# mrinmoy-iitg/SM_HPSS_MTL

Measured on AMD Instinct MI355X. Metric: clips/sec HPSS+MTL-CNN fwd (1s@16kHz), higher is better.
Workload: dtype f32

## Files before the change

### sm_hpss_mtl_amd/csrc/smh_fusion.hip

```cpp
#include "smh_model.h"
#include "smh_tcn_heads.h"

using namespace smh_tcn;

namespace {

constexpr int kFWaves = 16;
constexpr int kMaxMt = kPS / 16;

__device__ __forceinline__ f32x4 mfma4(float a, float b, f32x4 c) { return __builtin_amdgcn_mfma_f32_16x16x4f32(a, b, c, 0, 0, 0); }

template <bool TRAIN>
__global__ void __launch_bounds__(64 * kFWaves) fusion_dense_kernel(TcnArgs ta, int N, int D, const float *__restrict__ xh,
                                                                 const float *__restrict__ xp, const float *__restrict__ bn,
                                                                 const float *__restrict__ WhA, const float *__restrict__ hp,
                                                                 float *__restrict__ out) {
    extern __shared__ float part[];
    float *pre = part + (size_t)kFWaves * 16 * kPS;
    const int wave = __builtin_amdgcn_readfirstlane(threadIdx.x >> 6), lane = threadIdx.x & 63;
    const int i = lane & 15, q = lane >> 4;
    const int n0 = blockIdx.x * 16, g_here = min(16, N - n0);
    const int half = D / 2, ld = 64 * ((ta.NH + 63) / 64), n_mt = (ta.NH + 15) / 16;
    const int nr = min(n0 + i, N - 1);
    const float *gam = bn, *bet = bn + D, *mmean = bn + 2 * D, *mvar = bn + 3 * D;
    f32x4 acc[kMaxMt];
#pragma unroll
    for (int mt = 0; mt < kMaxMt; ++mt) acc[mt] = f32x4{0.f, 0.f, 0.f, 0.f};
    for (int c = wave; c < D / 16; c += kFWaves) {
        const int k = c * 16 + 4 * q;
        f32x4 av;
        const f32x4 g = *reinterpret_cast<const f32x4 *>(gam + k), b = *reinterpret_cast<const f32x4 *>(bet + k);
        if constexpr (TRAIN) {
            const f32x4 xv = *reinterpret_cast<const f32x4 *>(xh + (size_t)nr * D + k);
#pragma unroll
            for (int u = 0; u < 4; ++u) av[u] = xv[u] * g[u] + b[u];
        } else {
            const float *src = k < half ? xh + (size_t)nr * half + k : xp + (size_t)nr * half + (k - half);
            const f32x4 xv = *reinterpret_cast<const f32x4 *>(src);
            const f32x4 mm = *reinterpret_cast<const f32x4 *>(mmean + k), mv = *reinterpret_cast<const f32x4 *>(mvar + k);
#pragma unroll
            for (int u = 0; u < 4; ++u) av[u] = (xv[u] - mm[u]) / sqrtf(mv[u] + kBnEps) * g[u] + b[u];
        }
        const f32x4 *wrow = reinterpret_cast<const f32x4 *>(WhA) + (size_t)(c * 4 + q) * ld + i;
#pragma unroll
        for (int mt = 0; mt < kMaxMt; ++mt) {
            if (mt < n_mt) {
                const f32x4 bv = wrow[16 * mt];
#pragma unroll
                for (int u = 0; u < 4; ++u) acc[mt] = mfma4(av[u], bv[u], acc[mt]);
            }
        }
    }
#pragma unroll
    for (int mt = 0; mt < kMaxMt; ++mt)
        if (mt < n_mt)
#pragma unroll
            for (int r = 0; r < 4; ++r) part[((size_t)wave * 16 + 4 * q + r) * kPS + 16 * mt + i] = acc[mt][r];
    __syncthreads();
    for (int e = threadIdx.x; e < 16 * kPS; e += blockDim.x) {
        const int o = e % kPS;
        float v = 0.f;
        if (o < 16 * n_mt)
            for (int w = 0; w < kFWaves; ++w) v += part[(size_t)w * 16 * kPS + e];
        pre[e] = v;
    }
    __syncthreads();
    const float *bh = WhA + (size_t)D * ld;
    if constexpr (TRAIN) {
        for (int e = threadIdx.x; e < g_here * kPS; e += blockDim.x) {
            const int o = e % kPS;
            out[(size_t)n0 * kPS + e] = o < ta.NH ? pre[e] + bh[o] : 0.f;
        }
    } else {
        heads_tail(ta, pre, bh, hp, out, n0, g_here);
    }
}

constexpr int kFSlice = 32;
struct FusedAct {
    const float *acts[2];
    int nslot, half;
    __device__ __forceinline__ float pre_relu(int n, int k) const {
        const int b = k >= half, kk = k - b * half;
        return acts[b][((size_t)n * nslot + nslot - 1) * half + kk];
    }
};

__global__ void __launch_bounds__(256) fusion_bn_part_kernel(FusedAct fa, int N, int D, double *__restrict__ part) {
    const int k = blockIdx.x * 256 + threadIdx.x, s = blockIdx.y;
    if (k >= D) return;
    double s1 = 0.0, s2 = 0.0;
    for (int n = s * kFSlice; n < min(N, (s + 1) * kFSlice); ++n) {
        const double x = fmaxf(fa.pre_relu(n, k), 0.f);
        s1 += x, s2 += x * x;
    }
    part[((size_t)s * D + k) * 2] = s1;
    part[((size_t)s * D + k) * 2 + 1] = s2;
}

__global__ void __launch_bounds__(256) fusion_bn_final_kernel(int N, int D, int n_slices, const double *__restrict__ part,
// ... 11 lines not shown
__global__ void __launch_bounds__(256) fusion_bn_apply_kernel(FusedAct fa, int N, int D, const float *__restrict__ bnstat,
                                                              const float *__restrict__ vec, float *__restrict__ xhat) {
    const size_t e = (size_t)blockIdx.x * 256 + threadIdx.x;
    if (e >= (size_t)N * D) return;
    const int n = (int)(e / D), k = (int)(e - (size_t)n * D);
    xhat[e] = (fmaxf(fa.pre_relu(n, k), 0.f) - bnstat[k]) * vec[k];
}

struct FusionHeadOffs {
    size_t head[kMaxHeads];
};
__global__ void __launch_bounds__(256) fusion_dwh_kernel(int N, int D, int n_classes, const float *__restrict__ xhat,
                                                         const float *__restrict__ bn, const float *__restrict__ dpre,
                                                         float *__restrict__ grad, size_t off_c3, FusionHeadOffs offs) {
    const int wave = __builtin_amdgcn_readfirstlane(threadIdx.x >> 6), lane = threadIdx.x & 63;
    const int i = lane & 15, q = lane >> 4;
    const int k0 = (blockIdx.x * 4 + wave) * 16;
    if (k0 >= D) return;
    const int grp = blockIdx.y;
    const int ocount = grp == 0 ? n_classes : kHidden, col0 = grp == 0 ? 0 : n_classes + (grp - 1) * kHidden;
    const bool col_ok = i < ocount;
    const float g = bn[k0 + i], b = bn[D + k0 + i];
    f32x4 acc0 = {0.f, 0.f, 0.f, 0.f}, acc1 = acc0;
    for (int n = 0; n < N; n += 8) {
        float av[2], bv[2];
#pragma unroll
        for (int u = 0; u < 2; ++u) {
            const int nn = n + 4 * u + q;
            const bool ok = nn < N;
            const int nc = ok ? nn : 0;
            av[u] = ok ? xhat[(size_t)nc * D + k0 + i] * g + b : 0.f;
            bv[u] = (ok && col_ok) ? dpre[(size_t)nc * kPS + col0 + i] : 0.f;
        }
        acc0 = mfma4(av[0], bv[0], acc0);
        acc1 = mfma4(av[1], bv[1], acc1);
    }
    acc0 += acc1;
    if (col_ok) {
        const size_t base = (grp == 0 ? off_c3 : offs.head[grp - 1]) + (size_t)(k0 + 4 * q) * ocount + i;
#pragma unroll
        for (int r = 0; r < 4; ++r) grad[base + (size_t)r * ocount] = acc0[r];
    }
}

__global__ void __launch_bounds__(256) fusion_dx_kernel(int N, int D, int NH, const float *__restrict__ WhA,
                                                        const float *__restrict__ dpre, const float *__restrict__ xhat,
                                                        float *__restrict__ dy, double *__restrict__ part) {
    __shared__ float dp[kFSlice * kPS];
    const int k = blockIdx.x * 256 + threadIdx.x, s = blockIdx.y;
    const int nlo = s * kFSlice, nn = min(N, nlo + kFSlice) - nlo;
    for (int e = threadIdx.x; e < nn * kPS; e += 256) dp[e] = dpre[(size_t)nlo * kPS + e];
    __syncthreads();
    if (k >= D) return;
    const int ld = 64 * ((NH + 63) / 64);
    const float *w = WhA + (size_t)(k / 4) * ld * 4 + (k % 4);
    float acc[kFSlice];
#pragma unroll
    for (int r = 0; r < kFSlice; ++r) acc[r] = 0.f;
    for (int o = 0; o < NH; ++o) {
        const float wv = w[(size_t)o * 4];
#pragma unroll
        for (int r = 0; r < kFSlice; ++r) acc[r] = fmaf(dp[r * kPS + o], wv, acc[r]);
    }
    double s1 = 0.0, s2 = 0.0;
#pragma unroll
    for (int r = 0; r < kFSlice; ++r)
        if (r < nn) {
            const size_t e = (size_t)(nlo + r) * D + k;
            dy[e] = acc[r];
            s1 += acc[r];
            s2 += (double)acc[r] * xhat[e];
        }
    part[((size_t)s * D + k) * 2] = s1;
    part[((size_t)s * D + k) * 2 + 1] = s2;
}

__global__ void __launch_bounds__(256) fusion_bn_bwd_final_kernel(int N, int D, int n_slices, const double *__restrict__ part,
                                                                  float *__restrict__ grad, size_t off_bn, float *__restrict__ vec) {
    const int k = blockIdx.x * 256 + threadIdx.x;
    if (k >= D) return;
    double s1 = 0.0, s2 = 0.0;
    for (int s = 0; s < n_slices; ++s) s1 += part[((size_t)s * D + k) * 2], s2 += part[((size_t)s * D + k) * 2 + 1];
    grad[off_bn + k] = (float)s2;
    grad[off_bn + D + k] = (float)s1;
    vec[D + k] = (float)(s1 / N);
    vec[2 * D + k] = (float)(s2 / N);
}

__global__ void __launch_bounds__(256) fusion_bn_bwd_apply_kernel(FusedAct fa, int N, int D, const float *__restrict__ bn,
                                                                  const float *__restrict__ vec, const float *__restrict__ dy,
                                                                  const float *__restrict__ xhat, float *__restrict__ gt) {
    const size_t e = (size_t)blockIdx.x * 256 + threadIdx.x;
    if (e >= (size_t)N * D) return;
    const int n = (int)(e / D), k = (int)(e - (size_t)n * D);
    const int b = k >= fa.half, kk = k - b * fa.half;
    const float g = bn[k] * vec[k] * (dy[e] - vec[D + k] - xhat[e] * vec[2 * D + k]);
    gt[((size_t)b * N + n) * fa.half + kk] = fa.pre_relu(n, k) > 0.f ? g : 0.f;
}

}

namespace smh_tcn {

void fusion_tail_args(const smh_model *m, TcnArgs *a) {
    *a = TcnArgs{};
    a->D = m->D, a->NH = m->NH, a->n_mt = m->n_mt, a->n_classes = m->cfg.n_classes, a->n_heads = m->n_heads, a->out_dim = m->out_dim;
    for (int i = 0; i < kMaxHeads; ++i) a->head_odim[i] = m->head_odim[i], a->head_sigmoid[i] = m->head_sigmoid[i];
// ... 167 lines not shown
```

### sm_hpss_mtl_amd/csrc/smh_model.h

```cpp
#pragma once
#include "smh_common.h"

namespace smh_tcn {

using f32x4 = __attribute__((ext_vector_type(4))) float;

constexpr int C = 32;
constexpr int SX = 36;
constexpr int kMaxHeads = 4;
constexpr int kHidden = 16;
constexpr int kMaxG = 16;
constexpr int kPS = 80;
constexpr float kNormEps = 1e-5f;
constexpr float kBnEps = 1e-3f;
constexpr int kCat = kHidden + 2;
constexpr int kCatTail = 4 * kHidden + 4 * kCat + kCat + 1;
constexpr int kBlockFloats = 24 * 2 * 64 + 8 * 2 * 64 + 32 + 32;

struct TcnArgs {
    int N, T, F, FQ, G, GRP, n_blocks, n_dil, vec_ok;
    int D, NH, n_mt, n_classes, n_heads, out_dim, skip_heads;
    int wlds;
    unsigned long long *trace;
    int tune;
    int *status;
    int spin_limit;
    int split_last;
    int from_x0;
    int x0_shift, x0_T;
    int head_odim[kMaxHeads];
    int head_sigmoid[kMaxHeads];
    int cascade;
    int single;
    int trunk_only;
    int x0_one;
    const float *pair_X, *pair_W0, *pair_Wb;
    float *pair_trunk;
    const float *pair_WhA, *pair_hp;
    float *pair_out;
    int *pair_status;
};

struct TrainIO {
    float *acts;
    const float *drop_tcn;
    float *pre;
    float *upre;
    int acts_last_only;
};

struct HeadsArgs {
    int N, D, NH, n_classes, n_heads, out_dim;
    int head_odim[kMaxHeads], head_sigmoid[kMaxHeads];
    float lw[kMaxHeads + 1];
    size_t goff_head[kMaxHeads];
    size_t goff_c3b;
    size_t hp_off[kMaxHeads];
    int ext_losses;
    int stamps;
};
int launch_heads_train(const HeadsArgs &a, const float *pre, const float *y, const float *hp, const float *drop, float *dpre,
                       float *dxh, float *grad, float *bnstat, float *losses, unsigned *ticket, hipStream_t st);
int launch_cascade_heads_train(const HeadsArgs &a, const float *pre, const float *y, const float *hp, const float *drop,
                               float *dpre, float *dxh, float *dr, float *grad, float *bnstat, float *losses, hipStream_t st);
int launch_single_head_train(const HeadsArgs &a, const float *pre, const float *y, float *dpre, float *grad, float *losses,
// ... 78 lines not shown
```

### sm_hpss_mtl_amd/csrc/smh_tcn.hip

```cpp
#include <algorithm>
#include <cmath>
#include <cstdlib>
#include <cstring>
#include <type_traits>
#include <vector>

#include "smh_model.h"
#include "smh_tcn_heads.h"

using namespace smh_tcn;

namespace {

__device__ __forceinline__ f32x4 mfma4(float a, float b, f32x4 c) {
    return __builtin_amdgcn_mfma_f32_16x16x4f32(a, b, c, 0, 0, 0);
}

__device__ __forceinline__ float quad_max(float v) {
    const unsigned u = __float_as_uint(v);
    const auto r32 = __builtin_amdgcn_permlane32_swap(u, u, false, false);
    const float a = fmaxf(__uint_as_float(r32[0]), __uint_as_float(r32[1]));
    const unsigned ua = __float_as_uint(a);
    const auto r16 = __builtin_amdgcn_permlane16_swap(ua, ua, false, false);
    return fmaxf(__uint_as_float(r16[0]), __uint_as_float(r16[1]));
// ... 747 lines not shown
                    }
                    staged = blk + 2;
                    stage_ring(staged, 0, 1);
                }
                one_task(LdsWeights{ws + (size_t)(blk & (kWeightRing - 1)) * kBlockFloats, lane, q});
            }
        }
        publish();
        xin = (a.n_blocks & 1) ? xb : xa;
        xout = (a.n_blocks & 1) ? xa : xb;
        if (tracing && blockIdx.x < 1024 && threadIdx.x == 0) {
            a.trace[4 * (2000 + blockIdx.x) + 2] = __builtin_amdgcn_s_memtime();
            a.trace[4 * (2000 + blockIdx.x) + 3] = __builtin_amdgcn_s_memrealtime();
        }
    } else if (a.wlds && MODE == kPrefetch) {
        BlockW w0, w1;
        stage(0);
        if (a.n_blocks > 1) stage(1);
        asm volatile("s_waitcnt vmcnt(0)" ::: "memory");
        __syncthreads();
        load_block_lds(w0, ws, lane, q);
        for (int blk = 0; blk < a.n_blocks; blk += 2) {
            asm volatile("s_waitcnt vmcnt(0)" ::: "memory");
            __syncthreads();
            if (blk + 2 < a.n_blocks) stage(blk + 2);
            const bool more1 = blk + 1 < a.n_blocks;
            one_block(blk, w0, WeightPrefetch{w1, ws + kBlockFloats, lane, q});
            if (!more1) break;
            asm volatile("s_waitcnt vmcnt(0)" ::: "memory");
            __syncthreads();
            if (blk + 3 < a.n_blocks) stage(blk + 3);
            one_block(blk + 1, w1, WeightPrefetch{w0, ws, lane, q});
        }
    } else {
        if (a.wlds) stage(0);
        BlockW w;
        for (int blk = 0; blk < a.n_blocks; ++blk) {
            if (a.wlds) {
                asm volatile("s_waitcnt vmcnt(0)" ::: "memory");
                __syncthreads();
                if (blk + 1 < a.n_blocks) stage(blk + 1);
                one_block(blk, w, WeightLoad{w, ws + (size_t)(blk & 1) * kBlockFloats, lane, q});
            } else {
                __syncthreads();
                load_block_lds(w, Wb + (size_t)blk * kBlockFloats, lane, q);
                one_block(blk, w, NoPrefetch());
            }
        }
    }
    if (MODE != kSkew && MODE != kSkew16 && tracing && blockIdx.x < 1024 && threadIdx.x == 0) {
        a.trace[4 * (2000 + blockIdx.x) + 2] = __builtin_amdgcn_s_memtime();
        a.trace[4 * (2000 + blockIdx.x) + 3] = __builtin_amdgcn_s_memrealtime();
    }
    __syncthreads();
    if constexpr (MODE != kSkew && MODE != kSkew16) save_acts(xin, a.n_blocks);
    if constexpr (TRAIN) __syncthreads();
    for (int i = threadIdx.x; i < GR * (C / 4); i += blockDim.x) {
        const int R = i >> 3, c4 = (i & 7) * 4;
        f32x4 v = *reinterpret_cast<const f32x4 *>(xin + (size_t)R * SX + c4);
#pragma unroll
        for (int r = 0; r < 4; ++r) v[r] = fmaxf(v[r], 0.f);
        *reinterpret_cast<f32x4 *>(xin + (size_t)R * SX + c4) = v;
        if (trunk) *reinterpret_cast<f32x4 *>(trunk + ((size_t)n0 * T + R) * C + c4) = v;
    }
    __syncthreads();

    bool gave_up = false;
    if constexpr (MODE == kSkew || MODE == kSkew16) gave_up = ((__attribute__((address_space(3))) volatile int *)(flagbase))[63] != 0;
    dense_and_heads<TRAIN>(a, xin, xout, WhA, hp, out, tio, n0, g_here);
    if (tracing && blockIdx.x < 256 && threadIdx.x == 0) a.trace[4 * 3000 + 2 * blockIdx.x + 1] = __builtin_amdgcn_s_memrealtime();
    if (gave_up) {
        __syncthreads();
        for (int i = threadIdx.x; i < (a.trunk_only ? 0 : g_here * a.out_dim); i += blockDim.x) out[(size_t)n0 * a.out_dim + i] = 0.f;
        if (threadIdx.x == 0 && status) atomicOr(status, 1);
    }
}

__global__ void repack_kernel(const float *__restrict__ flat, const int *__restrict__ map, float *__restrict__ dst, size_t n) {
    const size_t i = (size_t)blockIdx.x * blockDim.x + threadIdx.x;
    if (i < n) {
        const int m = map[i];
        dst[i] = m ? flat[m - 1] : 0.f;
    }
}

static void pack_host(const smh_model *m, const float *h, std::vector<float> &W0, std::vector<float> &Wb,
                      std::vector<float> &WhA, std::vector<float> &hp) {
    const int F = m->cfg.n_feat, FQ = m->FQ, D = m->D, NH = m->NH, ncls = m->cfg.n_classes;
    W0.assign(m->nW0, 0.f), Wb.assign(m->nWb, 0.f), WhA.assign(m->nWhA, 0.f), hp.assign(m->nhp, 0.f);
    std::vector<float> Wh((size_t)D * NH, 0.f), bhv((size_t)m->n_mt * 16, 0.f);
    const float *p = h;
    if (m->heads == SMH_HEADS_FUSION) {
        p += 2 * trunk_floats(m->cfg) + (size_t)4 * D;
    } else if (m->cfg.block_variant == 1) {
        p += trunk_floats_v2(m->cfg);
    } else {
    for (int s = 0; s < FQ; ++s)
        for (int mt = 0; mt < 2; ++mt)
            for (int lane = 0; lane < 64; ++lane) {
                const int q = lane >> 4, i = lane & 15, f = q * FQ + s;
                W0[((size_t)s * 2 + mt) * 64 + lane] = f < F ? p[(size_t)f * C + 16 * mt + i] : 0.f;
            }
    p += (size_t)F * C;
    std::memcpy(&W0[(size_t)FQ * 2 * 64], p, C * sizeof(float));
    p += C;
    for (int b = 0; b < m->n_blocks; ++b) {
        float *wb = &Wb[(size_t)b * kBlockFloats];
        const float *k1 = p;
        p += 3 * C * C;
        const float *b1 = p;
        p += C;
        const float *k2 = p;
        p += C * C;
        const float *b2 = p;
        p += C;
        for (int s = 0; s < 24; ++s)
            for (int mt = 0; mt < 2; ++mt)
                for (int lane = 0; lane < 64; ++lane) {
                    const int q = lane >> 4, i = lane & 15;
                    const int tap = s / 8, c = 8 * q + s % 8;
                    const int n = s * 2 + mt;
                    wb[(n / 4) * 256 + 4 * lane + n % 4] = k1[((size_t)tap * C + c) * C + 16 * mt + i];
                }
        for (int e = 0; e < 8; ++e)
            for (int mt = 0; mt < 2; ++mt)
                for (int lane = 0; lane < 64; ++lane) {
                    const int q = lane >> 4, i = lane & 15;
                    const int cin = 16 * (e / 4) + 4 * q + (e % 4);
                    const int n = 48 + e * 2 + mt;
                    wb[(n / 4) * 256 + 4 * lane + n % 4] = k2[(size_t)cin * C + 16 * mt + i];
                }
        std::memcpy(wb + 24 * 2 * 64 + 8 * 2 * 64, b1, C * sizeof(float));
        std::memcpy(wb + 24 * 2 * 64 + 8 * 2 * 64 + 32, b2, C * sizeof(float));
    }
    }
    const float *k3c = p;
    p += (size_t)D * ncls;
    const float *b3c = p;
    p += ncls;
    for (int i = 0; i < D; ++i)
        for (int c = 0; c < ncls; ++c) Wh[(size_t)i * NH + c] = k3c[(size_t)i * ncls + c];
    for (int c = 0; c < ncls; ++c) bhv[c] = b3c[c];
    float *php = hp.data();
    for (int hd = 0; hd < m->n_heads; ++hd) {
        const float *kd = p;
        p += (size_t)D * kHidden;
        const float *bd = p;
        p += kHidden;
        for (int i = 0; i < D; ++i)
            for (int c = 0; c < kHidden; ++c) Wh[(size_t)i * NH + ncls + hd * kHidden + c] = kd[(size_t)i * kHidden + c];
        for (int c = 0; c < kHidden; ++c) bhv[ncls + hd * kHidden + c] = bd[c];
        const size_t cnt = head_tail_floats(m, hd);
        std::memcpy(php, p, cnt * sizeof(float));
        php += cnt;
        p += cnt;
    }
    const int ld = 64 * ((NH + 63) / 64);
    for (int k = 0; k < D; ++k)
        for (int o = 0; o < NH; ++o) WhA[(size_t)(k / 4) * ld * 4 + (size_t)o * 4 + (k % 4)] = Wh[(size_t)k * NH + o];
    std::memcpy(&WhA[(size_t)D * ld], bhv.data(), bhv.size() * sizeof(float));
}

}

static unsigned long long *g_trace = nullptr;
static unsigned g_trace_launches = 0;
constexpr size_t kTraceWords = 4 * 4096;
extern "C" int smh_internal_tcn_trace(int enable, unsigned long long *host, size_t words) {
    if (enable && !g_trace) {
        if (hipMalloc((void **)&g_trace, 2 * kTraceWords * sizeof(unsigned long long)) != hipSuccess) return -1;
        (void)hipMemset(g_trace, 0, 2 * kTraceWords * sizeof(unsigned long long));
    }
    if (host && g_trace) {
        (void)hipDeviceSynchronize();
        if (hipMemcpy(host, g_trace, std::min(words, 2 * kTraceWords) * sizeof(unsigned long long), hipMemcpyDeviceToHost) != hipSuccess) return -1;
    }
    if (!enable && g_trace) {
        (void)hipFree(g_trace);
        g_trace = nullptr;
    }
    return 0;
}

namespace smh_tcn {

Offsets offsets(const smh_model *m) {
    Offsets o;
    const size_t F = m->cfg.n_feat, D = m->D, ncls = m->cfg.n_classes;
    size_t p = 0;
    for (int h = 0; h < kMaxHeads; ++h) o.head[h] = 0;
    o.w0_k = p, p += F * C;
    o.w0_b = p, p += C;
    o.blk0 = p, o.blk_stride = 3 * C * C + C + C * C + C;
    p += (size_t)m->n_blocks * o.blk_stride;
    if (m->heads == SMH_HEADS_FUSION) {
        o.trunk_p = p, p += trunk_floats(m->cfg);
        o.fbn = p, p += 4 * D;
    }
    o.c3_k = p, p += D * ncls;
    o.c3_b = p, p += ncls;
    for (int h = 0; h < m->n_heads; ++h) {
        o.head[h] = p;
        p += D * kHidden + kHidden + head_tail_floats(m, h);
    }
    return o;
}

int repack(smh_model *m, hipStream_t st) {
    m->version++;
    if (m->heads == SMH_HEADS_FUSION) {
// ... 164 lines not shown
    SMH_REQUIRE(heads != SMH_HEADS_SINGLE || cfg->block_variant == 0,
                "smh_model_create_heads: the single-task model is built for block_variant 0 (keras-tcn 2.3.x) only");
    SMH_REQUIRE(heads != SMH_HEADS_FUSION || cfg->block_variant == 0,
                "smh_model_create_heads: the intermediate-fusion model is built for block_variant 0 (keras-tcn 2.3.x) only");
    SMH_REQUIRE(cfg->nb_filters == C, "B3_MTL kernel is tiled for nb_filters=32 (got %d)", cfg->nb_filters);
    SMH_REQUIRE(cfg->kernel_size == 3, "B3_MTL kernel supports kernel_size=3 (got %d)", cfg->kernel_size);
    if (heads == SMH_HEADS_SINGLE)
        SMH_REQUIRE(cfg->n_classes == 2 || cfg->n_classes == 3 || cfg->n_classes == 5,
                    "smh_model_create_heads: a single-task model has n_classes 2, 3 or 5 (got %d)", cfg->n_classes);
    else
        SMH_REQUIRE(cfg->n_classes == 3 || cfg->n_classes == 5, "n_classes must be 3 or 5 (got %d)", cfg->n_classes);
    SMH_REQUIRE(cfg->n_feat >= 1 && cfg->patch_size >= 1 && cfg->patch_size <= 512, "bad n_feat/patch_size");
    SMH_REQUIRE(cfg->nb_stacks >= 1 && cfg->n_dilations >= 1 && cfg->n_dilations <= 16, "bad stacks/dilations");
    SMH_REQUIRE(smh_device_count() > 0, "no HIP device visible: libsmh has no CPU path");
    smh_model *m = new smh_model();
    m->cfg = *cfg;
    m->n_blocks = cfg->nb_stacks * cfg->n_dilations;
    m->heads = heads;
    for (int i = 0; i < kMaxHeads; ++i) m->head_cat[i] = 0, m->head_odim[i] = 0, m->head_sigmoid[i] = 0;
    if (heads == SMH_HEADS_SINGLE) {
        m->n_heads = 0;
    } else if (heads == SMH_HEADS_CASCADED) {
        m->n_heads = 3;
        const int od[3] = {1, 1, 2}, sg[3] = {1, 1, 0};
        for (int i = 0; i < 3; ++i) m->head_odim[i] = od[i], m->head_sigmoid[i] = sg[i];
        m->head_cat[0] = m->head_cat[1] = kCat;
    } else if (cfg->n_classes == 5) {
        m->n_heads = 4;
        const int od[4] = {1, 1, 1, 3}, sg[4] = {1, 1, 1, 0};
        for (int i = 0; i < 4; ++i) m->head_odim[i] = od[i], m->head_sigmoid[i] = sg[i];
    } else {
        m->n_heads = 3;
        const int od[3] = {1, 1, 2}, sg[3] = {1, 1, 0};
        for (int i = 0; i < 3; ++i) m->head_odim[i] = od[i], m->head_sigmoid[i] = sg[i];
    }
    m->D = cfg->patch_size * C * (heads == SMH_HEADS_FUSION ? 2 : 1);
    m->NH = cfg->n_classes + kHidden * m->n_heads;
    m->n_mt = (m->NH + 15) / 16;
    m->out_dim = cfg->n_classes;
    for (int i = 0; i < m->n_heads; ++i) m->out_dim += m->head_odim[i];
    m->FQ = (cfg->n_feat + 3) / 4;
    SMH_REQUIRE(cfg->block_variant == 0 || cfg->block_variant == 1, "block_variant must be 0 (keras-tcn 2.3.x) or 1 (>= 2.8)");
    size_t n = (size_t)cfg->n_feat * C + C;
    n += (size_t)m->n_blocks * (3 * C * C + C + C * C + C);
    if (cfg->block_variant == 1) n = trunk_floats_v2(*cfg);
    if (heads == SMH_HEADS_FUSION) n = 2 * trunk_floats(*cfg) + (size_t)4 * m->D;
    n += (size_t)m->D * cfg->n_classes + cfg->n_classes;
    for (int i = 0; i < m->n_heads; ++i) n += (size_t)m->D * kHidden + kHidden + head_tail_floats(m, i);
    m->n_params = n;
    SMH_REQUIRE(n < (1u << 24), "model too large for the float-encoded gather map");
    m->nW0 = (size_t)m->FQ * 2 * 64 + 32;
    m->nWb = (size_t)m->n_blocks * kBlockFloats;
    if (cfg->block_variant == 1 || heads == SMH_HEADS_FUSION) m->nW0 = m->nWb = 0;
    m->nWhA = (size_t)m->D * 64 * ((m->NH + 63) / 64) + (size_t)m->n_mt * 16;
    m->nhp = 0;
    for (int i = 0; i < m->n_heads; ++i) m->nhp += head_tail_floats(m, i);
    std::vector<float> iota(n), W0, Wb, WhA, hp;
    for (size_t i = 0; i < n; ++i) iota[i] = (float)(i + 1);
    pack_host(m, iota.data(), W0, Wb, WhA, hp);
    std::vector<int> map;
    map.reserve(m->nW0 + m->nWb + m->nWhA + m->nhp);
    for (auto *v : {&W0, &Wb, &WhA, &hp})
        for (float f : *v) map.push_back((int)f);
    const size_t npk = map.size();
    hipError_t e = hipMalloc((void **)&m->d_flat, n * sizeof(float));
    if (e == hipSuccess) e = hipMalloc((void **)&m->d_W0, npk * sizeof(float));
    if (e == hipSuccess) e = hipMalloc((void **)&m->d_map, npk * sizeof(int));
    if (e == hipSuccess) e = hipMemcpy(m->d_map, map.data(), npk * sizeof(int), hipMemcpyHostToDevice);
    if (e == hipSuccess) e = hipMemset(m->d_flat, 0, n * sizeof(float));
    if (e == hipSuccess) e = hipMalloc((void **)&m->d_status, sizeof(int));
    if (e == hipSuccess) e = hipMemset(m->d_status, 0, sizeof(int));
    if (e == hipSuccess && heads == SMH_HEADS_FUSION) e = hipMalloc((void **)&m->d_w0cat, (size_t)2 * cfg->n_feat * C * sizeof(float));
    if (e == hipSuccess && heads == SMH_HEADS_FUSION) e = hipMemset(m->d_w0cat, 0, (size_t)2 * cfg->n_feat * C * sizeof(float));
    if (e != hipSuccess) {
        smh_model_destroy(m);
        return smh::set_error(SMH_E_HIP, "smh_model_create: device allocation failed: %s", hipGetErrorString(e));
    }
    m->d_Wb = m->d_W0 + m->nW0;
    m->d_WhA = m->d_Wb + m->nWb;
    m->d_hp = m->d_WhA + m->nWhA;
    if (heads == SMH_HEADS_FUSION) {
        for (int b = 0; b < 2; ++b) {
            const int rc = smh_model_create_heads(cfg, SMH_HEADS_MTL, &m->trunk[b]);
            if (rc) {
                smh_model_destroy(m);
                return rc;
            }
        }
    }
    *out = m;
    return SMH_OK;
}

extern "C" void smh_model_destroy(smh_model *m) {
    if (!m) return;
    (void)hipFree(m->d_flat);
    (void)hipFree(m->d_W0);
    (void)hipFree(m->d_map);
    (void)hipFree(m->d_bf16);
    (void)hipFree(m->d_status);
    (void)hipFree(m->d_w0cat);
    smh_model_destroy(m->trunk[0]);
    smh_model_destroy(m->trunk[1]);
    delete m;
}

extern "C" int smh_model_status(smh_model *m, void *stream) {
// ... 225 lines not shown
```

### sm_hpss_mtl_amd/csrc/smh_tcn_heads.h

```cpp
#pragma once
#include <type_traits>

#include "smh_model.h"

namespace smh_tcn {

__device__ __forceinline__ void cascaded_r(const TcnArgs &a, const float *pp, const float *bh, const float *hp, float r[2]) {
    const float *ph = hp + 2 * kCatTail;
    const float *gamma = ph, *beta = ph + 16, *mean = ph + 32, *var = ph + 48, *wo = ph + 64, *bo = wo + 2 * kHidden;
    r[0] = bo[0], r[1] = bo[1];
#pragma unroll
    for (int i = 0; i < kHidden; ++i) {
        const int o = a.n_classes + 2 * kHidden + i;
        float v = pp[o] + bh[o];
        v = (v - mean[i]) / sqrtf(var[i] + kBnEps);
        v = fmaxf(v * gamma[i] + beta[i], 0.f);
        r[0] = fmaf(v, wo[2 * i], r[0]);
        r[1] = fmaf(v, wo[2 * i + 1], r[1]);
    }
}

__device__ __forceinline__ void cascaded_head(const TcnArgs &a, const float *pp, const float *bh, const float *hp, float *orow, int h) {
    float r[2];
    cascaded_r(a, pp, bh, hp, r);
// ... 38 lines not shown
        }
        const float *gamma = ph, *beta = ph + 16, *mean = ph + 32, *var = ph + 48, *wo = ph + 64;
        const int od = a.head_odim[h];
        const float *bo = wo + kHidden * od;
        float hid[kHidden];
#pragma unroll
        for (int i = 0; i < kHidden; ++i) {
            const int o = a.n_classes + h * kHidden + i;
            float v = pre[p * kPS + o] + bh[o];
            v = (v - mean[i]) / sqrtf(var[i] + kBnEps);
            v = v * gamma[i] + beta[i];
            hid[i] = fmaxf(v, 0.f);
        }
        for (int c = 0; c < od; ++c) {
            float s = bo[c];
#pragma unroll
            for (int i = 0; i < kHidden; ++i) s = fmaf(hid[i], wo[i * od + c], s);
            if (a.head_sigmoid[h]) s = 1.0f / (1.0f + expf(-s));
            out[(size_t)(n0 + p) * a.out_dim + col + c] = s;
        }
    } else if (tid >= 128 && tid < 128 + g_here) {
        const int p = tid - 128;
        float mxl = -INFINITY;
        for (int c = 0; c < a.n_classes; ++c) mxl = fmaxf(mxl, pre[p * kPS + c] + bh[c]);
        float den = 0.f;
        for (int c = 0; c < a.n_classes; ++c) den += expf(pre[p * kPS + c] + bh[c] - mxl);
        const int col = a.out_dim - a.n_classes;
        for (int c = 0; c < a.n_classes; ++c)
            out[(size_t)(n0 + p) * a.out_dim + col + c] = expf(pre[p * kPS + c] + bh[c] - mxl) / den;
    }
}

__device__ __forceinline__ void single_tail(const TcnArgs &a, const float *pre, const float *bh, float *__restrict__ out, int n0,
                                            int g_here) {
    const int p = threadIdx.x;
    if (p >= g_here) return;
    constexpr int kMaxC = 5;
    float z[kMaxC], mx = -INFINITY, den = 0.f;
#pragma unroll
    for (int c = 0; c < kMaxC; ++c) {
        z[c] = c < a.n_classes ? pre[p * kPS + c] + bh[c] : -INFINITY;
        mx = fmaxf(mx, z[c]);
    }
#pragma unroll
    for (int c = 0; c < kMaxC; ++c) {
        z[c] = c < a.n_classes ? expf(z[c] - mx) : 0.f;
        den += z[c];
    }
#pragma unroll
    for (int c = 0; c < kMaxC; ++c)
        if (c < a.n_classes) out[(size_t)(n0 + p) * a.out_dim + c] = z[c] / den;
}

template <bool TRAIN>
__device__ __forceinline__ void dense_and_heads(const TcnArgs &a, const float *xin, float *xout, const float *__restrict__ WhA,
                                                const float *__restrict__ hp, float *__restrict__ out, const TrainIO &tio,
                                                int n0, int g_here) {
    if (a.trunk_only) return;
    const int wave = threadIdx.x >> 6, lane = threadIdx.x & 63, nw = blockDim.x >> 6;
    const int T = a.T;
    const int OPL = (a.NH + 63) >> 6;
    const int ld = OPL * 64;
    constexpr int kDenseParts = 8;
    float *part = xout;
    float *pre = xout + (size_t)kDenseParts * 4 * ld;
    const int rpp = (T + kDenseParts - 1) / kDenseParts;
    auto dense_on_trunk = [&](auto opl_c) {
        constexpr int kOPL = decltype(opl_c)::value;
        for (int g0 = 0; g0 < g_here; g0 += 4) {
            const float *xg[4];
#pragma unroll
            for (int g = 0; g < 4; ++g) xg[g] = xin + (size_t)min(g0 + g, g_here - 1) * T * SX;
            for (int pt = wave; pt < kDenseParts; pt += nw) {
                const int t_lo = min(T, pt * rpp), t_hi = min(T, t_lo + rpp);
                float acc[4][kOPL];
#pragma unroll
                for (int g = 0; g < 4; ++g)
#pragma unroll
                    for (int p = 0; p < kOPL; ++p) acc[g][p] = 0.f;
                for (int t = t_lo; t < t_hi; ++t) {
                    const f32x4 *wrow = reinterpret_cast<const f32x4 *>(WhA) + (size_t)t * (C / 4) * ld + lane;
#pragma unroll 2
                    for (int c8 = 0; c8 < 4; ++c8) {
                        f32x4 wa[kOPL], wb[kOPL];
#pragma unroll
                        for (int p = 0; p < kOPL; ++p) {
                            wa[p] = wrow[(size_t)(2 * c8) * ld + 64 * p];
                            wb[p] = wrow[(size_t)(2 * c8 + 1) * ld + 64 * p];
                        }
#pragma unroll
                        for (int g = 0; g < 4; ++g) {
                            const f32x4 xa = *reinterpret_cast<const f32x4 *>(xg[g] + (size_t)t * SX + 8 * c8);
                            const f32x4 xb = *reinterpret_cast<const f32x4 *>(xg[g] + (size_t)t * SX + 8 * c8 + 4);
#pragma unroll
                            for (int c = 0; c < 4; ++c)
#pragma unroll
                                for (int p = 0; p < kOPL; ++p) {
                                    acc[g][p] = fmaf(xa[c], wa[p][c], acc[g][p]);
                                    acc[g][p] = fmaf(xb[c], wb[p][c], acc[g][p]);
                                }
                        }
                    }
                }
#pragma unroll
                for (int g = 0; g < 4; ++g)
#pragma unroll
                    for (int p = 0; p < kOPL; ++p) part[((size_t)pt * 4 + g) * ld + 64 * p + lane] = acc[g][p];
            }
            __syncthreads();
            for (int i = threadIdx.x; i < 4 * ld; i += blockDim.x) {
                const int g = i / ld, o = i - g * ld;
                if (g0 + g < g_here && o < kPS) {
                    float v = 0.f;
#pragma unroll
                    for (int pt = 0; pt < kDenseParts; ++pt) v += part[((size_t)pt * 4 + g) * ld + o];
                    pre[(g0 + g) * kPS + o] = v;
                }
            }
            __syncthreads();
        }
    };
    if (!a.skip_heads) {
        if (OPL == 1) dense_on_trunk(std::integral_constant<int, 1>{});
        else dense_on_trunk(std::integral_constant<int, 2>{});
    }
    const float *bh = WhA + (size_t)a.D * ld;
    if constexpr (TRAIN) {
        for (int i = threadIdx.x; i < g_here * kPS; i += blockDim.x) {
            const int p = i / kPS, o = i - p * kPS;
            tio.pre[(size_t)(n0 + p) * kPS + o] = o < a.NH ? pre[p * kPS + o] + bh[o] : 0.f;
        }
        return;
    }
    if (a.single) single_tail(a, pre, bh, out, n0, g_here);
    else heads_tail(a, pre, bh, hp, out, n0, g_here);
}

}
```

### sm_hpss_mtl_amd/csrc/smh_tcn_v2.hip

```cpp
#include <algorithm>
#include <cstdlib>

#include "smh_model.h"
#include "smh_tcn_heads.h"

using namespace smh_tcn;

namespace {

__device__ __forceinline__ f32x4 mfma4(float a, float b, f32x4 c) { return __builtin_amdgcn_mfma_f32_16x16x4f32(a, b, c, 0, 0, 0); }

struct ConvW {
    float w[24][2];
    f32x4 blo, bhi;
};

__device__ __forceinline__ void load_conv(ConvW &cw, const float *__restrict__ k, const float *__restrict__ b, int q, int i) {
#pragma unroll
    for (int tap = 0; tap < 3; ++tap)
#pragma unroll
        for (int s8 = 0; s8 < 8; ++s8) {
            const float *p = k + ((size_t)tap * C + 8 * q + s8) * C + i;
            cw.w[tap * 8 + s8][0] = p[0];
            cw.w[tap * 8 + s8][1] = p[16];
// ... 93 lines not shown
                }
            } else {
                const float *xr = X + ((size_t)(n0 + g) * T + t) * C + 4 * q;
#pragma unroll
                for (int r = 0; r < 4; ++r) s0[r] = xr[r], s1[r] = xr[16 + r];
            }
#pragma unroll
            for (int r = 0; r < 4; ++r) {
                s0[r] = fmaxf(s0[r] + fmaxf(y0[r], 0.f), 0.f);
                s1[r] = fmaxf(s1[r] + fmaxf(y1[r], 0.f), 0.f);
            }
            float *dst = xa + (size_t)R * SX + 4 * q;
            *reinterpret_cast<f32x4 *>(dst) = s0;
            *reinterpret_cast<f32x4 *>(dst + 16) = s1;
        }
    }
    for (int blk = 1; blk < a.n_blocks; ++blk) {
        const int d = 1 << (blk % a.n_dil);
        const float *k0 = flat + blk0_floats + (size_t)(blk - 1) * blk_floats;
        const float *k1 = k0 + 3 * C * C + C;
        ConvW cw;
        load_conv(cw, k0, k0 + 3 * C * C, q, j);
        __syncthreads();
        for (int u = wave; u < units; u += nw) {
            const int R = 16 * u + j, Rc = min(R, GR - 1);
            const int t = Rc % T;
            f32x4 y0, y1;
            conv_tile(cw, xa, Rc, t, d, T, ZR, q, y0, y1);
#pragma unroll
            for (int r = 0; r < 4; ++r) y0[r] = fmaxf(y0[r], 0.f), y1[r] = fmaxf(y1[r], 0.f);
            float *dst = ya + (size_t)R * SX + 4 * q;
            *reinterpret_cast<f32x4 *>(dst) = y0;
            *reinterpret_cast<f32x4 *>(dst + 16) = y1;
        }
        load_conv(cw, k1, k1 + 3 * C * C, q, j);
        __syncthreads();
        for (int u = wave; u < units; u += nw) {
            const int R = 16 * u + j, Rc = min(R, GR - 1);
            const int t = Rc % T;
            f32x4 y0, y1;
            conv_tile(cw, ya, Rc, t, d, T, ZR, q, y0, y1);
            float *xr = xa + (size_t)Rc * SX + 4 * q;
            f32x4 s0 = *reinterpret_cast<const f32x4 *>(xr), s1 = *reinterpret_cast<const f32x4 *>(xr + 16);
#pragma unroll
            for (int r = 0; r < 4; ++r) {
                s0[r] = fmaxf(s0[r] + fmaxf(y0[r], 0.f), 0.f);
                s1[r] = fmaxf(s1[r] + fmaxf(y1[r], 0.f), 0.f);
            }
            float *dst = xa + (size_t)R * SX + 4 * q;
            *reinterpret_cast<f32x4 *>(dst) = s0;
            *reinterpret_cast<f32x4 *>(dst + 16) = s1;
        }
    }
    __syncthreads();
    if (trunk)
        for (int i = threadIdx.x; i < GR * (C / 4); i += blockDim.x) {
            const int R = i >> 3, c4 = (i & 7) * 4;
            *reinterpret_cast<f32x4 *>(trunk + ((size_t)n0 * T + R) * C + c4) = *reinterpret_cast<const f32x4 *>(xa + (size_t)R * SX + c4);
        }
    TrainIO none{nullptr, nullptr, nullptr, nullptr};
    dense_and_heads<false>(a, xa, ya, WhA, hp, out, none, n0, g_here);
}

}

namespace smh_tcn {

int launch_forward_v2(const smh_model *m, const float *d_x, int N, float *d_out, float *d_trunk, hipStream_t st) {
    TcnArgs a;
    size_t lds;
    fill_args(m, N, &a, &lds);
    lds = sizeof(float) * 2 * (size_t)(a.GRP + 1) * SX;
    SMH_REQUIRE(lds <= 156 * 1024, "patch_size %d too long for the LDS-resident TCN", a.T);
    const dim3 grid((N + a.G - 1) / a.G), block(512);
    SMH_CHECK_HIP(hipFuncSetAttribute((const void *)b3mtl_forward_v2_kernel, hipFuncAttributeMaxDynamicSharedMemorySize, (int)lds));
    hipLaunchKernelGGL(b3mtl_forward_v2_kernel, grid, block, lds, st, a, d_x, (const float *)m->d_flat, (const float *)m->d_WhA,
                       (const float *)m->d_hp, d_trunk, d_out);
    return smh::launch_status("b3mtl_forward_v2_kernel");
}

}
```

Before: 2.663 million.

## Software-pipeline dense-head weight loads with buffer loads, prefetch ring and packed layout

```diff
diff --git a/sm_hpss_mtl_amd/csrc/smh_fusion.hip b/sm_hpss_mtl_amd/csrc/smh_fusion.hip
--- a/sm_hpss_mtl_amd/csrc/smh_fusion.hip
+++ b/sm_hpss_mtl_amd/csrc/smh_fusion.hip
@@ -20,7 +20,7 @@
     const int wave = __builtin_amdgcn_readfirstlane(threadIdx.x >> 6), lane = threadIdx.x & 63;
     const int i = lane & 15, q = lane >> 4;
     const int n0 = blockIdx.x * 16, g_here = min(16, N - n0);
-    const int half = D / 2, ld = 64 * ((ta.NH + 63) / 64), n_mt = (ta.NH + 15) / 16;
+    const int half = D / 2, ld = dense_ld(ta.NH), n_mt = (ta.NH + 15) / 16;
     const int nr = min(n0 + i, N - 1);
     const float *gam = bn, *bet = bn + D, *mmean = bn + 2 * D, *mvar = bn + 3 * D;
     f32x4 acc[kMaxMt];
@@ -41,11 +41,11 @@
 #pragma unroll
             for (int u = 0; u < 4; ++u) av[u] = (xv[u] - mm[u]) / sqrtf(mv[u] + kBnEps) * g[u] + b[u];
         }
-        const f32x4 *wrow = reinterpret_cast<const f32x4 *>(WhA) + (size_t)(c * 4 + q) * ld + i;
+        const f32x4 *wrow = reinterpret_cast<const f32x4 *>(WhA) + (size_t)(c * 4 + q) * ld;
 #pragma unroll
         for (int mt = 0; mt < kMaxMt; ++mt) {
             if (mt < n_mt) {
-                const f32x4 bv = wrow[16 * mt];
+                const f32x4 bv = wrow[min(16 * mt + i, ta.NH - 1)];
 #pragma unroll
                 for (int u = 0; u < 4; ++u) acc[mt] = mfma4(av[u], bv[u], acc[mt]);
             }
@@ -163,7 +163,7 @@
     for (int e = threadIdx.x; e < nn * kPS; e += 256) dp[e] = dpre[(size_t)nlo * kPS + e];
     __syncthreads();
     if (k >= D) return;
-    const int ld = 64 * ((NH + 63) / 64);
+    const int ld = dense_ld(NH);
     const float *w = WhA + (size_t)(k / 4) * ld * 4 + (k % 4);
     float acc[kFSlice];
 #pragma unroll
diff --git a/sm_hpss_mtl_amd/csrc/smh_model.h b/sm_hpss_mtl_amd/csrc/smh_model.h
--- a/sm_hpss_mtl_amd/csrc/smh_model.h
+++ b/sm_hpss_mtl_amd/csrc/smh_model.h
@@ -11,6 +11,7 @@
 constexpr int kHidden = 16;
 constexpr int kMaxG = 16;
 constexpr int kPS = 80;
+__host__ __device__ constexpr int dense_ld(int NH) { return (NH + 3) & ~3; }
 constexpr float kNormEps = 1e-5f;
 constexpr float kBnEps = 1e-3f;
 constexpr int kCat = kHidden + 2;
diff --git a/sm_hpss_mtl_amd/csrc/smh_tcn.hip b/sm_hpss_mtl_amd/csrc/smh_tcn.hip
--- a/sm_hpss_mtl_amd/csrc/smh_tcn.hip
+++ b/sm_hpss_mtl_amd/csrc/smh_tcn.hip
@@ -823,6 +823,9 @@
         a.trace[4 * (2000 + blockIdx.x) + 2] = __builtin_amdgcn_s_memtime();
         a.trace[4 * (2000 + blockIdx.x) + 3] = __builtin_amdgcn_s_memrealtime();
     }
+    constexpr int kRows = MODE == kOneSet ? 2 : kDenseRows;
+    DenseFirst<kRows> dense_first;
+    dense_prefetch(a, WhA, dense_first);
     __syncthreads();
     if constexpr (MODE != kSkew && MODE != kSkew16) save_acts(xin, a.n_blocks);
     if constexpr (TRAIN) __syncthreads();
@@ -838,7 +841,7 @@
 
     bool gave_up = false;
     if constexpr (MODE == kSkew || MODE == kSkew16) gave_up = ((__attribute__((address_space(3))) volatile int *)(flagbase))[63] != 0;
-    dense_and_heads<TRAIN>(a, xin, xout, WhA, hp, out, tio, n0, g_here);
+    dense_and_heads<TRAIN, kRows>(a, xin, xout, WhA, hp, out, tio, n0, g_here, dense_first);
     if (tracing && blockIdx.x < 256 && threadIdx.x == 0) a.trace[4 * 3000 + 2 * blockIdx.x + 1] = __builtin_amdgcn_s_memrealtime();
     if (gave_up) {
         __syncthreads();
@@ -926,7 +929,7 @@
         php += cnt;
         p += cnt;
     }
-    const int ld = 64 * ((NH + 63) / 64);
+    const int ld = dense_ld(NH);
     for (int k = 0; k < D; ++k)
         for (int o = 0; o < NH; ++o) WhA[(size_t)(k / 4) * ld * 4 + (size_t)o * 4 + (k % 4)] = Wh[(size_t)k * NH + o];
     std::memcpy(&WhA[(size_t)D * ld], bhv.data(), bhv.size() * sizeof(float));
@@ -1197,7 +1200,7 @@
     m->nW0 = (size_t)m->FQ * 2 * 64 + 32;
     m->nWb = (size_t)m->n_blocks * kBlockFloats;
     if (cfg->block_variant == 1 || heads == SMH_HEADS_FUSION) m->nW0 = m->nWb = 0;
-    m->nWhA = (size_t)m->D * 64 * ((m->NH + 63) / 64) + (size_t)m->n_mt * 16;
+    m->nWhA = (size_t)m->D * dense_ld(m->NH) + (size_t)m->n_mt * 16;
     m->nhp = 0;
     for (int i = 0; i < m->n_heads; ++i) m->nhp += head_tail_floats(m, i);
     std::vector<float> iota(n), W0, Wb, WhA, hp;
diff --git a/sm_hpss_mtl_amd/csrc/smh_tcn_heads.h b/sm_hpss_mtl_amd/csrc/smh_tcn_heads.h
--- a/sm_hpss_mtl_amd/csrc/smh_tcn_heads.h
+++ b/sm_hpss_mtl_amd/csrc/smh_tcn_heads.h
@@ -114,42 +114,104 @@
         if (c < a.n_classes) out[(size_t)(n0 + p) * a.out_dim + c] = z[c] / den;
 }
 
-template <bool TRAIN>
+constexpr int kDenseParts = 8;
+constexpr int kDenseRows = 8;
+
+template <int OPL, int ROWS>
+struct DenseRing {
+    f32x4 w[OPL][ROWS];
+};
+template <int ROWS>
+using DenseFirst = DenseRing<2, ROWS>;
+
+typedef unsigned u32x4 __attribute__((ext_vector_type(4)));
+__device__ __forceinline__ unsigned dense_col(int NH, int lane, int p) { return 16u * (unsigned)min(64 * p + lane, NH - 1); }
+__device__ __forceinline__ __amdgpu_buffer_rsrc_t dense_rsrc(const float *WhA, int D, int ldc) {
+    return __builtin_amdgcn_make_buffer_rsrc(const_cast<float *>(WhA), 0, 4u * (unsigned)D * (unsigned)ldc, 0x00020000);
+}
+template <int OPL, int ROWS, int N>
+__device__ __forceinline__ void dense_load_pair(f32x4 (&w)[N][ROWS], __amdgpu_buffer_rsrc_t rw, int ldc, int t, int c8,
+                                                const unsigned *coff) {
+    static_assert(ROWS == 2 || ROWS == 4 || ROWS == 8, "ring slots: 2, 4 or 8 rows");
+    const unsigned rowb = 16u * (unsigned)ldc;
+#pragma unroll
+    for (int r = 0; r < 2; ++r)
+#pragma unroll
+        for (int p = 0; p < OPL; ++p) {
+            const u32x4 v = __builtin_amdgcn_raw_buffer_load_b128(rw, coff[p], ((unsigned)t * (C / 4) + 2 * c8 + r) * rowb, 0);
+            w[p][(2 * c8 + r) % ROWS] = f32x4{__uint_as_float(v.x), __uint_as_float(v.y), __uint_as_float(v.z), __uint_as_float(v.w)};
+        }
+}
+
+__device__ __forceinline__ void dense_range(int T, int pt, int &t_lo, int &t_hi) {
+    const int rpp = (T + kDenseParts - 1) / kDenseParts;
+    t_lo = min(T, pt * rpp), t_hi = min(T, t_lo + rpp);
+}
+
+template <int ROWS>
+__device__ __forceinline__ void dense_prefetch(const TcnArgs &a, const float *__restrict__ WhA, DenseFirst<ROWS> &first) {
+    const int wave = __builtin_amdgcn_readfirstlane(threadIdx.x >> 6), lane = threadIdx.x & 63;
+    int t_lo, t_hi;
+    dense_range(a.T, wave, t_lo, t_hi);
+    if (a.trunk_only || a.skip_heads || wave >= kDenseParts || t_lo >= t_hi) return;
+    const unsigned col[2] = {dense_col(a.NH, lane, 0), dense_col(a.NH, lane, 1)};
+    const int ldc = dense_ld(a.NH);
+    const __amdgpu_buffer_rsrc_t rw = dense_rsrc(WhA, a.D, ldc);
+    if (a.NH <= 64) {
+#pragma unroll
+        for (int c8 = 0; c8 < ROWS / 2; ++c8) dense_load_pair<1>(first.w, rw, ldc, t_lo, c8, col);
+    } else {
+#pragma unroll
+        for (int c8 = 0; c8 < ROWS / 2; ++c8) dense_load_pair<2>(first.w, rw, ldc, t_lo, c8, col);
+    }
+}
+
+template <bool TRAIN, int ROWS>
 __device__ __forceinline__ void dense_and_heads(const TcnArgs &a, const float *xin, float *xout, const float *__restrict__ WhA,
                                                 const float *__restrict__ hp, float *__restrict__ out, const TrainIO &tio,
-                                                int n0, int g_here) {
+                                                int n0, int g_here, const DenseFirst<ROWS> &first) {
     if (a.trunk_only) return;
-    const int wave = threadIdx.x >> 6, lane = threadIdx.x & 63, nw = blockDim.x >> 6;
+    const int wave = __builtin_amdgcn_readfirstlane(threadIdx.x >> 6), lane = threadIdx.x & 63, nw = blockDim.x >> 6;
     const int T = a.T;
     const int OPL = (a.NH + 63) >> 6;
-    const int ld = OPL * 64;
-    constexpr int kDenseParts = 8;
+    const int ldc = dense_ld(a.NH);
+    const int pl = OPL * 64;
     float *part = xout;
-    float *pre = xout + (size_t)kDenseParts * 4 * ld;
-    const int rpp = (T + kDenseParts - 1) / kDenseParts;
+    float *pre = xout + (size_t)kDenseParts * 4 * pl;
+    const __amdgpu_buffer_rsrc_t rw = dense_rsrc(WhA, a.D, ldc);
     auto dense_on_trunk = [&](auto opl_c) {
         constexpr int kOPL = decltype(opl_c)::value;
+        unsigned col[kOPL];
+#pragma unroll
+        for (int p = 0; p < kOPL; ++p) col[p] = dense_col(a.NH, lane, p);
+        DenseRing<kOPL, ROWS> f;
+#pragma unroll
+        for (int p = 0; p < kOPL; ++p)
+#pragma unroll
+            for (int h = 0; h < ROWS; ++h) f.w[p][h] = first.w[p][h];
         for (int g0 = 0; g0 < g_here; g0 += 4) {
             const float *xg[4];
 #pragma unroll
             for (int g = 0; g < 4; ++g) xg[g] = xin + (size_t)min(g0 + g, g_here - 1) * T * SX;
             for (int pt = wave; pt < kDenseParts; pt += nw) {
-                const int t_lo = min(T, pt * rpp), t_hi = min(T, t_lo + rpp);
+                int t_lo, t_hi;
+                dense_range(T, pt, t_lo, t_hi);
+                int t_next = -1;
+                {
+                    int npt = pt + nw, ng0 = g0, n_lo, n_hi;
+                    if (npt >= kDenseParts) npt = wave, ng0 = g0 + 4;
+                    dense_range(T, npt, n_lo, n_hi);
+                    if (ng0 < g_here && n_lo < n_hi) t_next = n_lo;
+                }
                 float acc[4][kOPL];
 #pragma unroll
                 for (int g = 0; g < 4; ++g)
 #pragma unroll
                     for (int p = 0; p < kOPL; ++p) acc[g][p] = 0.f;
-                for (int t = t_lo; t < t_hi; ++t) {
-                    const f32x4 *wrow = reinterpret_cast<const f32x4 *>(WhA) + (size_t)t * (C / 4) * ld + lane;
-#pragma unroll 2
+                auto frame = [&](int t, int nt, auto more_c) {
+                    constexpr bool MORE = decltype(more_c)::value;
+#pragma unroll
                     for (int c8 = 0; c8 < 4; ++c8) {
-                        f32x4 wa[kOPL], wb[kOPL];
-#pragma unroll
-                        for (int p = 0; p < kOPL; ++p) {
-                            wa[p] = wrow[(size_t)(2 * c8) * ld + 64 * p];
-                            wb[p] = wrow[(size_t)(2 * c8 + 1) * ld + 64 * p];
-                        }
 #pragma unroll
                         for (int g = 0; g < 4; ++g) {
                             const f32x4 xa = *reinterpret_cast<const f32x4 *>(xg[g] + (size_t)t * SX + 8 * c8);
@@ -158,24 +220,36 @@
                             for (int c = 0; c < 4; ++c)
 #pragma unroll
                                 for (int p = 0; p < kOPL; ++p) {
-                                    acc[g][p] = fmaf(xa[c], wa[p][c], acc[g][p]);
-                                    acc[g][p] = fmaf(xb[c], wb[p][c], acc[g][p]);
+                                    acc[g][p] = fmaf(xa[c], f.w[p][(2 * c8) % ROWS][c], acc[g][p]);
+                                    acc[g][p] = fmaf(xb[c], f.w[p][(2 * c8 + 1) % ROWS][c], acc[g][p]);
                                 }
                         }
+                        const int c8n = (c8 + ROWS / 2) & 3;
+                        const bool same = c8 + ROWS / 2 < 4;
+                        if (same || MORE) {
+                            __builtin_amdgcn_sched_barrier(0);
+                            dense_load_pair<kOPL>(f.w, rw, ldc, same ? t : nt, c8n, col);
+                            __builtin_amdgcn_sched_barrier(0);
+                        }
                     }
+                };
+                for (int t = t_lo; t + 1 < t_hi; ++t) frame(t, t + 1, std::true_type{});
+                if (t_lo < t_hi) {
+                    if (t_next >= 0) frame(t_hi - 1, t_next, std::true_type{});
+                    else frame(t_hi - 1, -1, std::false_type{});
                 }
 #pragma unroll
                 for (int g = 0; g < 4; ++g)
 #pragma unroll
-                    for (int p = 0; p < kOPL; ++p) part[((size_t)pt * 4 + g) * ld + 64 * p + lane] = acc[g][p];
+                    for (int p = 0; p < kOPL; ++p) part[((size_t)pt * 4 + g) * pl + 64 * p + lane] = acc[g][p];
             }
             __syncthreads();
-            for (int i = threadIdx.x; i < 4 * ld; i += blockDim.x) {
-                const int g = i / ld, o = i - g * ld;
+            for (int i = threadIdx.x; i < 4 * pl; i += blockDim.x) {
+                const int g = i / pl, o = i - g * pl;
                 if (g0 + g < g_here && o < kPS) {
                     float v = 0.f;
 #pragma unroll
-                    for (int pt = 0; pt < kDenseParts; ++pt) v += part[((size_t)pt * 4 + g) * ld + o];
+                    for (int pt = 0; pt < kDenseParts; ++pt) v += part[((size_t)pt * 4 + g) * pl + o];
                     pre[(g0 + g) * kPS + o] = v;
                 }
             }
@@ -186,7 +260,7 @@
         if (OPL == 1) dense_on_trunk(std::integral_constant<int, 1>{});
         else dense_on_trunk(std::integral_constant<int, 2>{});
     }
-    const float *bh = WhA + (size_t)a.D * ld;
+    const float *bh = WhA + (size_t)a.D * ldc;
     if constexpr (TRAIN) {
         for (int i = threadIdx.x; i < g_here * kPS; i += blockDim.x) {
             const int p = i / kPS, o = i - p * kPS;
diff --git a/sm_hpss_mtl_amd/csrc/smh_tcn_v2.hip b/sm_hpss_mtl_amd/csrc/smh_tcn_v2.hip
--- a/sm_hpss_mtl_amd/csrc/smh_tcn_v2.hip
+++ b/sm_hpss_mtl_amd/csrc/smh_tcn_v2.hip
@@ -169,6 +169,8 @@
             *reinterpret_cast<f32x4 *>(dst + 16) = s1;
         }
     }
+    DenseFirst<kDenseRows> dense_first;
+    dense_prefetch(a, WhA, dense_first);
     __syncthreads();
     if (trunk)
         for (int i = threadIdx.x; i < GR * (C / 4); i += blockDim.x) {
@@ -176,7 +178,7 @@
             *reinterpret_cast<f32x4 *>(trunk + ((size_t)n0 * T + R) * C + c4) = *reinterpret_cast<const f32x4 *>(xa + (size_t)R * SX + c4);
         }
     TrainIO none{nullptr, nullptr, nullptr, nullptr};
-    dense_and_heads<false>(a, xa, ya, WhA, hp, out, none, n0, g_here);
+    dense_and_heads<false, kDenseRows>(a, xa, ya, WhA, hp, out, none, n0, g_here, dense_first);
 }
 
 }
```

Result: no change. 2.658 million (-0.2%).
